# tpoisonooo/how-to-optimize-gemm

Hardware: NVIDIA H100
Metric: SGEMM GFLOP/s (square N=4096 point of the 256..4096 sweep) (higher is better)
Workload: dtype f16x2(scaled split-f32)

## Files before the change

how-to-optimize-gemm_b200/csrc/capi.cu:

```cuda
#include "../../include/b200gemm.h"

#include <cuda.h>
#include <cuda_runtime.h>
#include <stdio.h>
#include <stdlib.h>
#include <string.h>

#include <atomic>
#include <mutex>
#include <vector>

#include "gemm_ffma.cuh"
#include "gemm_generic.cuh"
#include "gemm_mxf4.cuh"
#include "gemm_tc.cuh"

using namespace b200;

namespace {

std::atomic<unsigned long long> g_launches{0};
int g_split_tail = 1;

struct KernelTimer {
// ... 2 lines not shown
  int n = 0;
  cudaEvent_t ev[CAP][2] = {};
  void begin(cudaStream_t st) {
    if (!on || n >= CAP) return;
    if (!ev[n][0]) { cudaEventCreate(&ev[n][0]); cudaEventCreate(&ev[n][1]); }
    cudaEventRecord(ev[n][0], st);
  }
  void end(cudaStream_t st) {
    if (!on || n >= CAP) return;
    cudaEventRecord(ev[n][1], st);
    n++;
  }
} g_ktimer;
std::atomic<int> g_default_f32_mode{-1};
thread_local const char* t_last_kernel = "none";
struct Schedule { int tiles = 0, split = 0, full_tiles = 0, ctas = 0; };
thread_local Schedule t_last_schedule;
int g_dbg_b_lbo = 0, g_dbg_b_sbo = 0;

struct Call {
  cudaStream_t st = nullptr;
  int acc = 0;
  int axpby = 0;
  float alpha = 1.f, beta = 0.f;
  const void* bias = nullptr;
  int act = -1;
  int sm_reserve = 0;
  bool epi() const { return act >= 0; }
};

constexpr int kFlagSlots = 16;
struct Scratch { void* p = nullptr; size_t bytes = 0; };
struct HostPipe {
  bool ready = false;
  cudaStream_t h2d = nullptr, comp = nullptr, d2h = nullptr;
  cudaEvent_t in[8] = {}, done[8] = {};
  cudaError_t init() {
    if (ready) return cudaSuccess;
    cudaError_t e;
    if ((e = cudaStreamCreateWithFlags(&h2d, cudaStreamNonBlocking)) != cudaSuccess) return e;
    if ((e = cudaStreamCreateWithFlags(&comp, cudaStreamNonBlocking)) != cudaSuccess) return e;
    if ((e = cudaStreamCreateWithFlags(&d2h, cudaStreamNonBlocking)) != cudaSuccess) return e;
    for (int i = 0; i < 8; i++) {
      if ((e = cudaEventCreateWithFlags(&in[i], cudaEventDisableTiming)) != cudaSuccess) return e;
      if ((e = cudaEventCreateWithFlags(&done[i], cudaEventDisableTiming)) != cudaSuccess) return e;
    }
    ready = true;
    return cudaSuccess;
  }
};
struct DevCtx {
  int ok = 0;
  int sms = 0;
  int dev = -1;
  int* flags = nullptr;
  std::mutex flag_mu;
  unsigned flag_slot = 0;
  struct FlagUser {
    cudaStream_t st = nullptr;
    cudaEvent_t ev = nullptr;
    bool used = false;
  } flag_user[kFlagSlots];
  std::mutex ws_mu;
  Scratch ws;
  cudaEvent_t ws_event = nullptr;
  cudaStream_t ws_stream = nullptr;
  bool ws_busy = false;
  struct MaxBuf {
    unsigned slot = 0;
    float* buf = nullptr;
    size_t cap = 0;
    int dirty[2] = {0, 0};
  } cmax, amax;
  cudaStream_t aux = nullptr;
  cudaEvent_t aux_fork = nullptr, aux_join = nullptr;
  std::mutex host_mu;
  Scratch scr[4];
  HostPipe pipe;
  std::vector<const void*> attr_done;
};
constexpr int kMaxDevices = 64;
DevCtx g_ctx[kMaxDevices];
std::mutex g_mu;

typedef CUresult (*EncodeTiledFn)(CUtensorMap*, CUtensorMapDataType, cuuint32_t, void*,
                                  const cuuint64_t*, const cuuint64_t*, const cuuint32_t*,
                                  const cuuint32_t*, CUtensorMapInterleave, CUtensorMapSwizzle,
                                  CUtensorMapL2promotion, CUtensorMapFloatOOBfill);
EncodeTiledFn g_encode = nullptr;

thread_local DevCtx* t_ctx = nullptr;
thread_local int t_bound_dev = -1;

int ensure_device() {
  int dev = -1;
  if (cudaGetDevice(&dev) != cudaSuccess || dev < 0 || dev >= kMaxDevices) { cudaGetLastError(); t_ctx = nullptr; return B200_ERR_NO_DEVICE; }
  if (t_bound_dev != dev) {
    if (cudaSetDevice(dev) != cudaSuccess) { cudaGetLastError(); t_ctx = nullptr; return B200_ERR_NO_DEVICE; }
    t_bound_dev = dev;
  }
  DevCtx* c = &g_ctx[dev];
  t_ctx = c;
  if (c->ok == 1) return 0;
  std::lock_guard<std::mutex> lk(g_mu);
  if (c->ok == 1) return 0;
  cudaDeviceProp prop;
  if (cudaGetDeviceProperties(&prop, dev) != cudaSuccess) { cudaGetLastError(); c->ok = -1; return B200_ERR_NO_DEVICE; }
  if (prop.major != 9) { c->ok = -1; return B200_ERR_NO_DEVICE; }
  if (!g_encode) {
    void* fn = nullptr;
    cudaDriverEntryPointQueryResult qres;
    if (cudaGetDriverEntryPoint("cuTensorMapEncodeTiled", &fn, cudaEnableDefault, &qres) != cudaSuccess ||
        qres != cudaDriverEntryPointSuccess || !fn) {
      cudaGetLastError();
      c->ok = -1;
      return B200_ERR_NO_DEVICE;
    }
    g_encode = reinterpret_cast<EncodeTiledFn>(fn);
  }
  if (!c->flags) {
    if (cudaMalloc(&c->flags, kFlagSlots * 1024 * sizeof(int)) != cudaSuccess ||
        cudaMemset(c->flags, 0, kFlagSlots * 1024 * sizeof(int)) != cudaSuccess) {
      cudaGetLastError(); c->flags = nullptr; c->ok = -1; return B200_ERR_NO_DEVICE;
    }
  }
  if (!c->ws_event && cudaEventCreateWithFlags(&c->ws_event, cudaEventDisableTiming) != cudaSuccess) {
    cudaGetLastError(); c->ok = -1; return B200_ERR_NO_DEVICE;
  }
  for (auto& u : c->flag_user)
    if (!u.ev && cudaEventCreateWithFlags(&u.ev, cudaEventDisableTiming) != cudaSuccess) {
      cudaGetLastError(); u.ev = nullptr; c->ok = -1; return B200_ERR_NO_DEVICE;
    }
  c->dev = dev;
  c->sms = prop.multiProcessorCount;
  c->ok = 1;
  return 0;
}

template <typename Kern>
int ensure_smem_attr(Kern kern, int bytes) {
  const void* key = reinterpret_cast<const void*>(kern);
  {
    std::lock_guard<std::mutex> lk(g_mu);
    for (const void* k : t_ctx->attr_done) if (k == key) return 0;
  }
  cudaError_t e = cudaFuncSetAttribute(kern, cudaFuncAttributeMaxDynamicSharedMemorySize, bytes);
  if (e != cudaSuccess) { cudaGetLastError(); return (int)e; }
  std::lock_guard<std::mutex> lk(g_mu);
  t_ctx->attr_done.push_back(key);
  return 0;
}

struct MapKey {
  const void* ptr; int dtype; unsigned long long d0, d1, ld_bytes; unsigned b0, b1; int swz; int dev;
  unsigned long long d2, d2_bytes;
  bool operator==(const MapKey& o) const {
    return ptr == o.ptr && dtype == o.dtype && d0 == o.d0 && d1 == o.d1 && ld_bytes == o.ld_bytes &&
           b0 == o.b0 && b1 == o.b1 && swz == o.swz && dev == o.dev && d2 == o.d2 && d2_bytes == o.d2_bytes;
  }
};
struct MapEntry { MapKey key; CUtensorMap map; };
std::vector<MapEntry> g_maps;
size_t g_map_next = 0;
constexpr size_t kMapCache = 64;

int get_map(CUtensorMap* out, const void* ptr, CUtensorMapDataType dt, int elem_bytes,
            unsigned long long inner, unsigned long long rows, unsigned long long ld_bytes,
            unsigned box_inner, unsigned box_rows, int swizzle ,
            unsigned long long entries = 0, unsigned long long entry_bytes = 0) {
  MapKey key{ptr, (int)dt, inner, rows, ld_bytes, box_inner, box_rows, swizzle, t_ctx->dev, entries, entry_bytes};
  std::lock_guard<std::mutex> lk(g_mu);
  for (auto& e : g_maps)
    if (e.key == key) { *out = e.map; return 0; }
  cuuint64_t dims[3] = {inner, rows, entries};
  cuuint64_t strides[2] = {ld_bytes, entry_bytes};
  cuuint32_t box[3] = {box_inner, box_rows, 1};
  cuuint32_t estr[3] = {1, 1, 1};
  CUtensorMap m;
  CUresult r = g_encode(&m, dt, entries ? 3 : 2, const_cast<void*>(ptr), dims, strides, box, estr,
                        CU_TENSOR_MAP_INTERLEAVE_NONE,
                        swizzle == 1 ? CU_TENSOR_MAP_SWIZZLE_128B
                        : swizzle == 2 ? CU_TENSOR_MAP_SWIZZLE_128B_ATOM_32B
                        : swizzle == 3 ? CU_TENSOR_MAP_SWIZZLE_64B : CU_TENSOR_MAP_SWIZZLE_NONE,
                        CU_TENSOR_MAP_L2_PROMOTION_L2_256B, CU_TENSOR_MAP_FLOAT_OOB_FILL_NONE);
  (void)elem_bytes;
  if (r != CUDA_SUCCESS) return B200_ERR_TENSORMAP;
  if (g_maps.size() < kMapCache) g_maps.push_back({key, m});
  else { g_maps[g_map_next] = {key, m}; g_map_next = (g_map_next + 1) % kMapCache; }
  *out = m;
  return 0;
}

inline bool aligned16(const void* p) { return (reinterpret_cast<uintptr_t>(p) & 15) == 0; }

int check_args(int m, int n, int k, const void* A, int lda, const void* B, int ldb, const void* C, int ldc,
               int op_a = B200_OP_N, int op_b = B200_OP_N) {
  if ((op_a != B200_OP_N && op_a != B200_OP_T) || (op_b != B200_OP_N && op_b != B200_OP_T)) return B200_ERR_BAD_ARG;
  if (m < 0 || n < 0 || k < 0) return B200_ERR_BAD_ARG;
  if (m == 0 || n == 0) return 1;
  if (!C || ldc < n) return B200_ERR_BAD_ARG;
  if (k > 0 && (!A || !B || lda < (op_a ? m : k) || ldb < (op_b ? k : n))) return B200_ERR_BAD_ARG;
  return 0;
}

int last_launch_status() {
  cudaError_t e = cudaPeekAtLastError();
  if (e != cudaSuccess) { cudaGetLastError(); return (int)e; }
  return 0;
}

int g_pdl = 1;
int g_prepass_fork = 1;
template <typename... KArgs, typename... Args>
cudaError_t launch_pdl(void (*kern)(KArgs...), dim3 grid, dim3 block, size_t smem, cudaStream_t st, int cluster, Args&&... args) {
  cudaLaunchConfig_t cfg = {};
  cfg.gridDim = grid; cfg.blockDim = block; cfg.dynamicSmemBytes = smem; cfg.stream = st;
  cudaLaunchAttribute at[2];
  int n = 0;
  if (cluster > 1) {
    at[n].id = cudaLaunchAttributeClusterDimension;
    at[n].val.clusterDim.x = cluster; at[n].val.clusterDim.y = 1; at[n].val.clusterDim.z = 1;
    n++;
  }
  if (g_pdl) {
    at[n].id = cudaLaunchAttributeProgrammaticStreamSerialization;
    at[n].val.programmaticStreamSerializationAllowed = 1;
    n++;
  }
  cfg.attrs = at; cfg.numAttrs = n;
  return cudaLaunchKernelEx(&cfg, kern, std::forward<Args>(args)...);
}

template <typename T>
int launch_zero(int m, int n, T* C, int ldc, cudaStream_t st) {
  dim3 grid((n + 255) / 256, m < 4096 ? m : 4096);
  fill_zero_kernel<T><<<grid, 256, 0, st>>>(m, n, C, ldc);
  g_launches++;
  t_last_kernel = "fill_zero";
  return last_launch_status();
}

template <typename InT, typename OutT>
int launch_generic(int op_a, int op_b, int m, int n, int k, const void* A, int lda, const void* B, int ldb, void* C,
                   int ldc, const char* name, const Call& c) {
  dim3 grid((n + 63) / 64, (m + 63) / 64);
  const long long a_rs = op_a ? 1 : lda, a_cs = op_a ? lda : 1, b_rs = op_b ? 1 : ldb, b_cs = op_b ? ldb : 1;
  gemm_generic_kernel<InT, OutT><<<grid, 256, 0, c.st>>>(m, n, k, static_cast<const InT*>(A), a_rs, a_cs,
                                                         static_cast<const InT*>(B), b_rs, b_cs, static_cast<OutT*>(C), ldc,
                                                         c.acc, nullptr, nullptr, c.axpby, c.alpha, c.beta,
                                                         static_cast<const InT*>(c.bias), c.act);
  g_launches++;
  t_last_kernel = name;
  return last_launch_status();
}

int launch_generic_requant(int m, int n, int k, const int8_t* A, int lda, const int8_t* B, int ldb, int8_t* C,
                           int ldc, const float* scales, const float* bias, cudaStream_t st) {
  dim3 grid((n + 63) / 64, (m + 63) / 64);
  gemm_generic_kernel<int8_t, int8_t><<<grid, 256, 0, st>>>(m, n, k, A, lda, 1, B, ldb, 1, C, ldc, 0, scales, bias);
  g_launches++;
  t_last_kernel = "generic_s8_requant_64x64";
  return last_launch_status();
}

int take_flag_slot(cudaStream_t st, int** flags, DevCtx::FlagUser** user) {
// ... 351 lines not shown
  if (ws.rc) return ws.rc;
  uint16_t* pA = reinterpret_cast<uint16_t*>(ws.base());
  const uint16_t* pB = prepB ? prepB : reinterpret_cast<uint16_t*>(ws.base() + round1024(ga.bytes(NP)));
  const SplitJob ja{A, lda, ga.rows, ga.cols, pA, ga.pitch, ga.plane_rows},
                 jb{B, ldb, gb.rows, gb.cols, const_cast<uint16_t*>(pB), gb.pitch, gb.plane_rows};
  if (int rc = launch_split<NP>(ja, jb, prepB ? 1 : 2, c.st)) return rc;
  using Prod = typename std::conditional<NP == 3, ProdX3, ProdX2>::type;
  return with_layout(op_a, op_b, [&](auto L) {
    using Lay = decltype(L);
    return launch_tc<KIND_F16, 128, NP == 3 ? 4 : 6, float, Prod, 64, Lay::AL, Lay::BL>(
        m, n, k, pA, ga.pitch, NP * ga.plane_rows, ga.plane_rows, pB, gb.pitch, NP * gb.plane_rows, gb.plane_rows, C, ldc,
        (NP == 3 ? kNamesBf16x3 : kNamesBf16x2)[Lay::idx][2], c, g_split_chunk_k[NP == 3 ? 0 : 1]);
  });
}

struct F16Operand {
  const uint16_t* planes;
  long long pitch;
  int plane_rows;
  const float* maxv;
};

int launch_f16_split_rows(const float* A, long long lda, int rows, int cols, float* rmax, uint16_t* planes,
                          long long pitch, int plane_rows, cudaStream_t st) {
  int blocks = (plane_rows + 7) / 8;
  const int cap = t_ctx->sms * 16;
  if (blocks > cap) blocks = cap;
  if (blocks < 1) blocks = 1;
  if (cols <= 1024) launch_pdl(split_f16_rows_kernel<4>, dim3(blocks), dim3(256), 0, st, 1, A, (long long)lda, rows, cols, rmax, planes, pitch, plane_rows);
  else if (cols <= 2048) launch_pdl(split_f16_rows_kernel<8>, dim3(blocks), dim3(256), 0, st, 1, A, (long long)lda, rows, cols, rmax, planes, pitch, plane_rows);
  else if (cols <= 4096) launch_pdl(split_f16_rows_kernel<16>, dim3(blocks), dim3(256), 0, st, 1, A, (long long)lda, rows, cols, rmax, planes, pitch, plane_rows);
  else launch_pdl(split_f16_rows_kernel<0>, dim3(blocks), dim3(256), 0, st, 1, A, (long long)lda, rows, cols, rmax, planes, pitch, plane_rows);
  g_launches++;
  return last_launch_status();
}

int launch_f16_split_cols(const float* B, long long ldb, int rows, int cols, float* cmax, uint16_t* planes,
                          long long pitch, int plane_rows, float* zero_buf, int zero_n, cudaStream_t st) {
  launch_pdl(col_absmax_kernel, dim3((cols + 1023) / 1024, (rows + 15) / 16), dim3(256), 0, st, 1, B, (long long)ldb, rows, cols,
             reinterpret_cast<unsigned int*>(cmax));
  const int gx = (int)((pitch + 2047) / 2048);
  int gy = (t_ctx->sms * 8 + gx - 1) / gx;
  if (gy > (plane_rows + 1) / 2) gy = (plane_rows + 1) / 2;
  if (gy < 1) gy = 1;
  if (zero_buf && zero_n > gx * 2048) {
    cudaMemsetAsync(zero_buf, 0, (size_t)zero_n * 4, st);
    zero_buf = nullptr;
  }
  launch_pdl(split_f16_cols_kernel, dim3(gx, gy), dim3(256), 0, st, 1, B, (long long)ldb, rows, cols, (const float*)cmax, planes, pitch, plane_rows, zero_buf, zero_n);
  g_launches += 2;
  return last_launch_status();
}

int gemm_f16x2_core(int op_a, int op_b, int m, int n, int k, const F16Operand& a, const F16Operand& b, float* C, int ldc,
                    const Call& c) {
  constexpr int NP = 2;
  return with_layout(op_a, op_b, [&](auto L) {
    using Lay = decltype(L);
    return launch_tc<KIND_FP16, 128, 6, float, ProdX2, 64, Lay::AL, Lay::BL>(
        m, n, k, a.planes, a.pitch, NP * a.plane_rows, a.plane_rows, b.planes, b.pitch, NP * b.plane_rows, b.plane_rows, C,
        ldc, kNamesF16x2[Lay::idx][2], c, g_split_chunk_k[2], a.maxv, b.maxv);
  });
}

int cmax_reserve(DevCtx::MaxBuf& mb, int n, float** cur, float** other, int* other_dirty) {
  if (mb.cap < (size_t)n) {
    size_t cap = mb.cap ? 2 * mb.cap : 16384;
    if (cap < (size_t)n) cap = (size_t)n;
    if (mb.buf) { cudaDeviceSynchronize(); cudaFree(mb.buf); }
    mb.buf = nullptr; mb.cap = 0;
    cudaError_t e = cudaMalloc(&mb.buf, 2 * cap * sizeof(float));
    if (e == cudaSuccess) e = cudaMemset(mb.buf, 0, 2 * cap * sizeof(float));
    if (e != cudaSuccess) { cudaGetLastError(); return (int)e; }
    mb.cap = cap;
    mb.dirty[0] = mb.dirty[1] = 0;
  }
  const unsigned slot = mb.slot++ & 1u;
  *cur = mb.buf + slot * mb.cap;
  *other = mb.buf + (slot ^ 1u) * mb.cap;
  *other_dirty = mb.dirty[slot ^ 1u];
  mb.dirty[slot ^ 1u] = 0;
  mb.dirty[slot] = n;
  return 0;
}

struct F16Ws {
  PlaneGeom ga, gb;
  size_t a_off, r_off, rb_off, total;
};
F16Ws f16x2_ws(int op_a, int op_b, int m, int n, int k, bool prepA, bool prepB) {
  F16Ws w{geom_a(op_a, m, k), geom_b(op_b, k, n)};
  w.a_off = round1024(prepA ? 0 : w.ga.bytes(2));
  w.r_off = round1024(w.a_off + (prepB ? 0 : w.gb.bytes(2)));
  const size_t ra = prepA || op_a ? 0 : (size_t)m * 4;
  w.rb_off = round1024(w.r_off + ra);
  w.total = prepB || !op_b ? w.r_off + ra : w.rb_off + (size_t)n * 4;
  return w;
}

int gemm_f32_split_f16(int op_a, int op_b, int m, int n, int k, const float* A, int lda, const float* B, int ldb, float* C,
                       int ldc, const F16Operand* prepA, const F16Operand* prepB, const Call& c) {
  if (prepA && prepB) return gemm_f16x2_core(B200_OP_N, B200_OP_N, m, n, k, *prepA, *prepB, C, ldc, c);
  const F16Ws w = f16x2_ws(op_a, op_b, m, n, k, prepA != nullptr, prepB != nullptr);
  const PlaneGeom &ga = w.ga, &gb = w.gb;
  WsLease ws(w.total, c.st);
  if (ws.rc) return ws.rc;
  uint8_t* base = ws.base();
  F16Operand oa, ob;
  DevCtx* dc = t_ctx;
  const bool fork = !prepA && !prepB && g_prepass_fork && (double)m * k + (double)k * n >= 4.0e6;
  cudaStream_t sb = c.st;
  if (fork) {
    if (!dc->aux) {
      if (cudaStreamCreateWithFlags(&dc->aux, cudaStreamNonBlocking) != cudaSuccess ||
          cudaEventCreateWithFlags(&dc->aux_fork, cudaEventDisableTiming) != cudaSuccess ||
          cudaEventCreateWithFlags(&dc->aux_join, cudaEventDisableTiming) != cudaSuccess) { cudaGetLastError(); return B200_ERR_NO_DEVICE; }
    }
    cudaEventRecord(dc->aux_fork, c.st);
    cudaStreamWaitEvent(dc->aux, dc->aux_fork, 0);
    sb = dc->aux;
  }
  if (prepB) ob = *prepB;
  else if (op_b) {
    uint16_t* pB = reinterpret_cast<uint16_t*>(base + w.a_off);
    float* bmax = reinterpret_cast<float*>(base + w.rb_off);
    if (int rc = launch_f16_split_rows(B, ldb, n, k, bmax, pB, gb.pitch, gb.plane_rows, sb)) return rc;
    ob = F16Operand{pB, gb.pitch, gb.plane_rows, bmax};
  } else {
    uint16_t* pB = reinterpret_cast<uint16_t*>(base + w.a_off);
    float *cmax, *other;
    int other_dirty;
    if (int rc = cmax_reserve(dc->cmax, n, &cmax, &other, &other_dirty)) return rc;
    if (int rc = launch_f16_split_cols(B, ldb, k, n, cmax, pB, gb.pitch, gb.plane_rows, other, other_dirty, sb)) return rc;
    ob = F16Operand{pB, gb.pitch, gb.plane_rows, cmax};
  }
  if (prepA) oa = *prepA;
  else if (op_a) {
    uint16_t* pA = reinterpret_cast<uint16_t*>(base);
    float *amax, *other;
    int other_dirty;
    if (int rc = cmax_reserve(dc->amax, m, &amax, &other, &other_dirty)) return rc;
    if (int rc = launch_f16_split_cols(A, lda, k, m, amax, pA, ga.pitch, ga.plane_rows, other, other_dirty, c.st)) return rc;
    oa = F16Operand{pA, ga.pitch, ga.plane_rows, amax};
  } else {
    uint16_t* pA = reinterpret_cast<uint16_t*>(base);
    float* rmax = reinterpret_cast<float*>(base + w.r_off);
    if (int rc = launch_f16_split_rows(A, lda, m, k, rmax, pA, ga.pitch, ga.plane_rows, c.st)) return rc;
    oa = F16Operand{pA, ga.pitch, ga.plane_rows, rmax};
  }
  if (fork) {
    cudaEventRecord(dc->aux_join, dc->aux);
    cudaStreamWaitEvent(c.st, dc->aux_join, 0);
  }
  return gemm_f16x2_core(op_a, op_b, m, n, k, oa, ob, C, ldc, c);
}

template <class Cfg, class Kern>
int launch_ffma(Kern kern, int ctas_per_sm, const char* name, int m, int n, int k, const float* A, int lda,
                const float* B, int ldb, float* C, int ldc, const Call& c) {
  CUtensorMap tmA, tmB;
  int rc = get_map(&tmA, A, CU_TENSOR_MAP_DATA_TYPE_FLOAT32, 4, k, m, (unsigned long long)lda * 4, Cfg::BK, Cfg::BM, 1);
  if (rc) return rc;
  rc = get_map(&tmB, B, CU_TENSOR_MAP_DATA_TYPE_FLOAT32, 4, n, k, (unsigned long long)ldb * 4, Cfg::BN, Cfg::BK, 0);
// ... 366 lines not shown
  if (k == 0 || alpha == 0.f) return c32 ? degenerate_grouped<float>(n, C, ldc, gr, c) : degenerate_grouped<E>(n, C, ldc, gr, c);
  if (!tma_ok(A, lda, B, ldb, 2) || (groups > 1 && !batch_tma_ok(stride_b, b_rows, ldb, 2))) {
    if (c32) return launch_generic_grouped<E, float>(op_b, n, k, A, lda, B, ldb, C, ldc, gr, K16::kGenericGrp, c);
    return launch_generic_grouped<E, E>(op_b, n, k, A, lda, B, ldb, C, ldc, gr, K16::kGenericGrp, c);
  }
  if (c32) return tc16_grouped<KIND, float>(op_b, n, k, A, lda, B, ldb, C, ldc, gr, c);
  return tc16_grouped<KIND, typename K16::Out16>(op_b, n, k, A, lda, B, ldb, C, ldc, gr, c);
}

static_assert(ACT_NONE == B200_ACT_NONE && ACT_RELU == B200_ACT_RELU && ACT_GELU == B200_ACT_GELU &&
              ACT_GELU_TANH == B200_ACT_GELU_TANH, "EpiAct follows the header's codes");

int gemm_s8(int op_a, int op_b, int m, int n, int k, const int8_t* A, int lda, const int8_t* B, int ldb, int32_t* C,
            int ldc, cudaStream_t st) {
  int rc = check_args(m, n, k, A, lda, B, ldb, C, ldc, op_a, op_b);
  if (rc == 1) return 0;
  if (rc) return rc;
  if ((rc = ensure_device())) return rc;
  Call c{st};
  if (k == 0) return launch_zero<int32_t>(m, n, C, ldc, st);
  if (!tma_ok(A, lda, B, ldb, 1))
    return launch_generic<int8_t, int32_t>(op_a, op_b, m, n, k, A, lda, B, ldb, C, ldc, "generic_s8_64x64", c);
  return tc_s8(op_a, op_b, m, n, k, A, lda, B, ldb, C, ldc, c);
}

}

extern "C" {

const char* b200_gemm_version(void) { return "b200gemm 0.3 (sm_90a; wgmma+TMA)"; }

int b200_gemm_device_ok(void) { return ensure_device(); }

const char* b200_gemm_strerror(int code) {
  switch (code) {
    case B200_OK: return "ok";
    case B200_ERR_BAD_ARG: return "bad argument";
    case B200_ERR_NO_DEVICE: return "no usable sm_90 CUDA device (there is no CPU fallback)";
    case B200_ERR_UNSUPPORTED: return "mode not supported for these operands";
    case B200_ERR_TENSORMAP: return "cuTensorMapEncodeTiled failed";
    case B200_ERR_NCCL: return "NCCL failure (b200_nccl_last_error has the text)";
    default: return code > 0 ? cudaGetErrorString((cudaError_t)code) : "unknown";
  }
}

const char* b200_gemm_last_kernel(void) { return t_last_kernel; }
unsigned long long b200_gemm_launch_count(void) { return g_launches.load(); }
int b200_gemm_default_f32_mode(void) { return resolve_f32_mode(B200_F32_AUTO); }
void b200_gemm_set_default_f32_mode(int mode) {
  if (mode >= 0 && mode != B200_F32_AUTO && mode <= B200_F32_F16X2) g_default_f32_mode.store(mode);
}
void b200_gemm_debug_set_b_desc(int lbo_bytes, int sbo_bytes) { g_dbg_b_lbo = lbo_bytes; g_dbg_b_sbo = sbo_bytes; }
void b200_gemm_debug_set_bn(int bn) { g_force_bn = bn; }
void b200_gemm_debug_set_pdl(int v) { g_pdl = (v & 1) != 0; g_prepass_fork = (v & 2) == 0; }
void b200_gemm_debug_set_dynamic_sched(int) {}
void b200_gemm_debug_set_cta_group(int) {}
void b200_gemm_debug_set_split_tail(int on) { g_split_tail = on; }
void b200_gemm_debug_last_schedule(int* tiles, int* split, int* full_tiles, int* ctas) {
  const Schedule& s = t_last_schedule;
  if (tiles) *tiles = s.tiles;
  if (split) *split = s.split;
  if (full_tiles) *full_tiles = s.full_tiles;
  if (ctas) *ctas = s.ctas;
}
void b200_gemm_debug_set_epilogue(int) {}
void b200_gemm_debug_set_group_rows(int rows) { g_group_rows = rows; }
void b200_gemm_debug_set_ffma_variant(int v) { g_ffma_halves = v & 1; g_ffma_fat = v < 0 ? -1 : (v >> 1) & 1; }
void b200_gemm_debug_set_split_chunk(int x3_k, int x2_k) {
  g_split_chunk_k[0] = x3_k < 0 ? kSplitChunkDefault[0] : x3_k;
  g_split_chunk_k[1] = x2_k < 0 ? kSplitChunkDefault[1] : x2_k;
  g_split_chunk_k[2] = x2_k < 0 ? kSplitChunkDefault[2] : x2_k;
}
void b200_gemm_debug_kernel_timing(int enable) { g_ktimer.on = enable != 0; g_ktimer.n = 0; }
int b200_gemm_debug_kernel_time_ms(double* sum_ms) {
  double sum = 0;
  int cnt = 0;
  for (int i = 0; i < g_ktimer.n; i++) {
    float ms = 0.f;
    if (cudaEventSynchronize(g_ktimer.ev[i][1]) == cudaSuccess &&
        cudaEventElapsedTime(&ms, g_ktimer.ev[i][0], g_ktimer.ev[i][1]) == cudaSuccess) { sum += ms; cnt++; }
  }
  cudaGetLastError();
  g_ktimer.n = 0;
  if (sum_ms) *sum_ms = sum;
  return cnt;
}

int b200_gemm_reserve_workspace(size_t bytes) {
  int rc = ensure_device();
  if (rc) return rc;
  std::lock_guard<std::mutex> wlk(t_ctx->ws_mu);
  return split_ws_reserve(bytes);
}
size_t b200_gemm_workspace_bytes_op(int op_a, int op_b, int m, int n, int k, int precision_mode) {
  if ((op_a != B200_OP_N && op_a != B200_OP_T) || (op_b != B200_OP_N && op_b != B200_OP_T)) return 0;
  if (m <= 0 || n <= 0 || k <= 0) return 0;
  size_t bytes = 0;
  for (int tma = 0; tma < 2; tma++)
    for (int general = 0; general < 2; general++) {
      const size_t b = f32_route_ws_bytes(f32_route(precision_mode, m, n, k, tma, general), op_a, op_b, m, n, k);
      if (b > bytes) bytes = b;
    }
  return bytes;
}
size_t b200_gemm_workspace_bytes(int m, int n, int k, int precision_mode) {
  return b200_gemm_workspace_bytes_op(B200_OP_N, B200_OP_N, m, n, k, precision_mode);
}
// ... 400 lines not shown
```

how-to-optimize-gemm_b200/csrc/gemm_tc.cuh:

```cuda
#pragma once
#include <cuda_fp16.h>
#include <string.h>
#include <type_traits>

#include "ptx.cuh"
#include "wgmma.cuh"

namespace b200 {

enum Layout { LAYOUT_K = 0, LAYOUT_MN = 1 };

template <int KIND> struct KindTraits;
template <> struct KindTraits<KIND_F16>  { static constexpr int ELEM = 2; static constexpr int B_LAYOUT = LAYOUT_MN; };
template <> struct KindTraits<KIND_FP16> { static constexpr int ELEM = 2; static constexpr int B_LAYOUT = LAYOUT_MN; };
template <> struct KindTraits<KIND_TF32> { static constexpr int ELEM = 4; static constexpr int B_LAYOUT = LAYOUT_K; };
template <> struct KindTraits<KIND_I8>   { static constexpr int ELEM = 1; static constexpr int B_LAYOUT = LAYOUT_K; };

struct ProdSingle {
  static constexpr int N = 1, NPA = 1, NPB = 1;
  __host__ __device__ static constexpr int ia(int) { return 0; }
  __host__ __device__ static constexpr int ib(int) { return 0; }
};
struct ProdX3 {
  static constexpr int N = 6, NPA = 3, NPB = 3;
// ... 813 lines not shown
          const float4 v0 = __ldcs(reinterpret_cast<const float4*>(s));
          const float4 v1 = __ldcs(reinterpret_cast<const float4*>(s) + 1);
          x[u][0] = v0.x; x[u][1] = v0.y; x[u][2] = v0.z; x[u][3] = v0.w;
          x[u][4] = v1.x; x[u][5] = v1.y; x[u][6] = v1.z; x[u][7] = v1.w;
        } else {
#pragma unroll
          for (int e = 0; e < 8; e++)
            if (c + e < cols) x[u][e] = s[e];
        }
      }
    }
#pragma unroll
    for (int u = 0; u < 2; u++) {
      const int r = r0 + u;
      if (r >= plane_rows) break;
#pragma unroll
      for (int pl = 0; pl < NP; pl++) {
        uint32_t w[4];
#pragma unroll
        for (int e = 0; e < 4; e++) w[e] = bf16_plane2(x[u][2 * e], x[u][2 * e + 1]);
        *reinterpret_cast<uint4*>(dst + ((long long)pl * plane_rows + r) * dld + c) = make_uint4(w[0], w[1], w[2], w[3]);
      }
    }
  }
}


__device__ __forceinline__ void split_f16x8(const float (&x)[8], uint4& h1, uint4& h2) {
  uint32_t a[4], b[4];
#pragma unroll
  for (int e = 0; e < 4; e++) {
    const __half2 p = __floats2half2_rn(x[2 * e], x[2 * e + 1]);
    const float2 pf = __half22float2(p);
    const __half2 q = __floats2half2_rn(x[2 * e] - pf.x, x[2 * e + 1] - pf.y);
    a[e] = *reinterpret_cast<const uint32_t*>(&p);
    b[e] = *reinterpret_cast<const uint32_t*>(&q);
  }
  h1 = make_uint4(a[0], a[1], a[2], a[3]);
  h2 = make_uint4(b[0], b[1], b[2], b[3]);
}
__device__ __forceinline__ void load8(const float* __restrict__ s, int c, int cols, bool vec, float (&x)[8]) {
  if (vec && c + 8 <= cols) {
    const float4 v0 = __ldg(reinterpret_cast<const float4*>(s + c));
    const float4 v1 = __ldg(reinterpret_cast<const float4*>(s + c) + 1);
    x[0] = v0.x; x[1] = v0.y; x[2] = v0.z; x[3] = v0.w;
    x[4] = v1.x; x[5] = v1.y; x[6] = v1.z; x[7] = v1.w;
  } else {
#pragma unroll
    for (int e = 0; e < 8; e++) x[e] = c + e < cols ? __ldg(s + c + e) : 0.f;
  }
}

template <int VPL>
__global__ void __launch_bounds__(256) split_f16_rows_kernel(const float* __restrict__ src, long long ld, int rows,
                                                             int cols, float* __restrict__ rmax,
                                                             uint16_t* __restrict__ dst, long long dld, int plane_rows) {
  griddep_launch();
  griddep_wait();
  const int lane = threadIdx.x & 31;
  const int nwarps = (gridDim.x * blockDim.x) >> 5;
  const bool vec = (ld & 3) == 0 && (reinterpret_cast<uintptr_t>(src) & 15) == 0;
  for (int r = (blockIdx.x * blockDim.x + threadIdx.x) >> 5; r < plane_rows; r += nwarps) {
    uint16_t* d1 = dst + (long long)r * dld;
    uint16_t* d2 = dst + ((long long)plane_rows + r) * dld;
    if (r >= rows) {
      for (int c = lane * 8; c < dld; c += 256) {
        *reinterpret_cast<uint4*>(d1 + c) = make_uint4(0, 0, 0, 0);
        *reinterpret_cast<uint4*>(d2 + c) = make_uint4(0, 0, 0, 0);
      }
      continue;
    }
    const float* s = src + (long long)r * ld;
    float mx = 0.f;
    if constexpr (VPL > 0) {
      float x[VPL][8];
#pragma unroll
      for (int j = 0; j < VPL; j++) {
        const int c = (j * 32 + lane) * 8;
#pragma unroll
        for (int e = 0; e < 8; e++) x[j][e] = 0.f;
        if (c < cols) load8(s, c, cols, vec, x[j]);
#pragma unroll
        for (int e = 0; e < 8; e++) mx = fmaxf(mx, fabsf(x[j][e]));
      }
#pragma unroll
      for (int o = 16; o > 0; o >>= 1) mx = fmaxf(mx, __shfl_xor_sync(0xffffffffu, mx, o));
      if (lane == 0) rmax[r] = mx;
      const int ex = -pow2_exp(mx);
#pragma unroll
      for (int j = 0; j < VPL; j++) {
        const int c = (j * 32 + lane) * 8;
        if (c < dld) {
#pragma unroll
          for (int e = 0; e < 8; e++) x[j][e] = scale_pow2(x[j][e], ex);
          uint4 h1, h2;
          split_f16x8(x[j], h1, h2);
          *reinterpret_cast<uint4*>(d1 + c) = h1;
          *reinterpret_cast<uint4*>(d2 + c) = h2;
        }
      }
    } else {
      for (int c0 = lane * 8; c0 < cols; c0 += 1024) {
        float x[4][8];
#pragma unroll
        for (int u = 0; u < 4; u++) {
          const int c = c0 + u * 256;
#pragma unroll
          for (int e = 0; e < 8; e++) x[u][e] = 0.f;
          if (c < cols) load8(s, c, cols, vec, x[u]);
#pragma unroll
          for (int e = 0; e < 8; e++) mx = fmaxf(mx, fabsf(x[u][e]));
        }
      }
#pragma unroll
      for (int o = 16; o > 0; o >>= 1) mx = fmaxf(mx, __shfl_xor_sync(0xffffffffu, mx, o));
      if (lane == 0) rmax[r] = mx;
      const int ex = -pow2_exp(mx);
      for (int c0 = lane * 8; c0 < dld; c0 += 512) {
        float x[2][8];
#pragma unroll
        for (int u = 0; u < 2; u++) {
          const int c = c0 + u * 256;
#pragma unroll
          for (int e = 0; e < 8; e++) x[u][e] = 0.f;
          if (c < cols) load8(s, c, cols, vec, x[u]);
        }
#pragma unroll
        for (int u = 0; u < 2; u++) {
          const int c = c0 + u * 256;
          if (c < dld) {
#pragma unroll
            for (int e = 0; e < 8; e++) x[u][e] = scale_pow2(x[u][e], ex);
            uint4 h1, h2;
            split_f16x8(x[u], h1, h2);
            *reinterpret_cast<uint4*>(d1 + c) = h1;
            *reinterpret_cast<uint4*>(d2 + c) = h2;
          }
        }
      }
    }
  }
}

__global__ void __launch_bounds__(256) col_absmax_kernel(const float* __restrict__ src, long long ld, int rows,
                                                         int cols, unsigned int* __restrict__ out) {
  constexpr int ROWS = 16;
  griddep_launch();
  griddep_wait();
  const int c = blockIdx.x * 1024 + threadIdx.x * 4;
  if (c >= cols) return;
  const int r0 = blockIdx.y * ROWS, r1 = min(r0 + ROWS, rows);
  const bool vec = (ld & 3) == 0 && (reinterpret_cast<uintptr_t>(src) & 15) == 0 && c + 4 <= cols;
  float4 mx = make_float4(0.f, 0.f, 0.f, 0.f);
  if (vec) {
#pragma unroll 16
    for (int r = r0; r < r1; r++) {
      const float4 v = __ldg(reinterpret_cast<const float4*>(src + (long long)r * ld + c));
      mx.x = fmaxf(mx.x, fabsf(v.x)); mx.y = fmaxf(mx.y, fabsf(v.y));
      mx.z = fmaxf(mx.z, fabsf(v.z)); mx.w = fmaxf(mx.w, fabsf(v.w));
    }
  } else {
    for (int r = r0; r < r1; r++) {
      const float* s = src + (long long)r * ld + c;
      mx.x = fmaxf(mx.x, fabsf(s[0]));
      if (c + 1 < cols) mx.y = fmaxf(mx.y, fabsf(s[1]));
      if (c + 2 < cols) mx.z = fmaxf(mx.z, fabsf(s[2]));
      if (c + 3 < cols) mx.w = fmaxf(mx.w, fabsf(s[3]));
    }
  }
  const float m4[4] = {mx.x, mx.y, mx.z, mx.w};
#pragma unroll
  for (int e = 0; e < 4; e++)
    if (c + e < cols && __float_as_uint(m4[e]) > __ldcg(out + c + e)) atomicMax(out + c + e, __float_as_uint(m4[e]));
}

__global__ void __launch_bounds__(256) split_f16_cols_kernel(const float* __restrict__ src, long long ld, int rows,
                                                             int cols, const float* __restrict__ cmax,
                                                             uint16_t* __restrict__ dst, long long dld, int plane_rows,
                                                             float* __restrict__ zero_buf, int zero_n) {
  griddep_launch();
  griddep_wait();
  const int c = (int)(blockIdx.x * 256 + threadIdx.x) * 8;
  if (blockIdx.y == 0 && zero_buf != nullptr) {
#pragma unroll
    for (int e = 0; e < 8; e++)
      if (c + e < zero_n) zero_buf[c + e] = 0.f;
  }
  if (c >= dld) return;
  const bool vec = (ld & 3) == 0 && (reinterpret_cast<uintptr_t>(src) & 15) == 0;
  int ex[8];
#pragma unroll
  for (int e = 0; e < 8; e++) ex[e] = c + e < cols ? -pow2_exp(__ldg(cmax + c + e)) : 0;
  for (int r0 = blockIdx.y * 2; r0 < plane_rows; r0 += gridDim.y * 2) {
    float x[2][8];
#pragma unroll
    for (int u = 0; u < 2; u++) {
      const int r = r0 + u;
#pragma unroll
      for (int e = 0; e < 8; e++) x[u][e] = 0.f;
      if (r < rows) load8(src + (long long)r * ld, c, cols, vec, x[u]);
    }
#pragma unroll
    for (int u = 0; u < 2; u++) {
      const int r = r0 + u;
      if (r >= plane_rows) break;
#pragma unroll
      for (int e = 0; e < 8; e++) x[u][e] = scale_pow2(x[u][e], ex[e]);
      uint4 h1, h2;
      split_f16x8(x[u], h1, h2);
      *reinterpret_cast<uint4*>(dst + (long long)r * dld + c) = h1;
      *reinterpret_cast<uint4*>(dst + ((long long)plane_rows + r) * dld + c) = h2;
    }
  }
}

}
```

how-to-optimize-gemm_b200/csrc/ptx.cuh:

```cuda
#pragma once
#include <cuda.h>
#include <cuda_runtime.h>
#include <math.h>
#include <stdint.h>

namespace b200 {

__device__ __forceinline__ uint32_t smem_u32(const void* p) {
  return static_cast<uint32_t>(__cvta_generic_to_shared(p));
}

__device__ __forceinline__ void mbar_init(uint32_t bar, uint32_t count) {
  asm volatile("mbarrier.init.shared::cta.b64 [%0], %1;" ::"r"(bar), "r"(count) : "memory");
}
__device__ __forceinline__ void fence_barrier_init() {
  asm volatile("fence.mbarrier_init.release.cluster;" ::: "memory");
}
__device__ __forceinline__ void fence_proxy_async() {
  asm volatile("fence.proxy.async.shared::cta;" ::: "memory");
}
__device__ __forceinline__ void mbar_arrive_expect_tx(uint32_t bar, uint32_t bytes) {
  asm volatile("mbarrier.arrive.expect_tx.shared::cta.b64 _, [%0], %1;" ::"r"(bar), "r"(bytes)
               : "memory");
}
// ... 44 lines not shown
      "cp.async.bulk.tensor.2d.shared::cluster.global.tile.mbarrier::complete_tx::bytes"
      ".L2::cache_hint [%0], [%1, {%3, %4}], [%2], %5;"
      ::"r"(dst_smem), "l"(reinterpret_cast<uint64_t>(m)), "r"(bar), "r"(c0), "r"(c1), "l"(policy)
      : "memory");
}

enum MmaKind { KIND_F16 = 0 , KIND_TF32 = 1, KIND_I8 = 2, KIND_FP16 = 3  };
enum Swz { SWZ_128B = 1, SWZ_64B = 2 };

__device__ __forceinline__ uint64_t make_sdesc(uint32_t smem_addr, uint32_t lbo_bytes, uint32_t sbo_bytes, uint32_t swz) {
  uint64_t d = 0;
  d |= (uint64_t)((smem_addr & 0x3FFFF) >> 4);
  d |= (uint64_t)((lbo_bytes >> 4) & 0x3FFF) << 16;
  d |= (uint64_t)((sbo_bytes >> 4) & 0x3FFF) << 32;
  d |= (uint64_t)swz << 62;
  return d;
}

__device__ __forceinline__ int32_t requant_s8(int32_t acc, float scale, float bias, bool has_bias) {
  float f = __fmul_rn(__int2float_rn(acc), scale);
  if (has_bias) f = __fadd_rn(f, bias);
  const float g = fminf(fmaxf(f, -200.0f), 200.0f);
  const float magic = 12582912.0f;
  float r = __fadd_rn(__fadd_rn(g, magic), -magic);
  if (fabsf(__fadd_rn(g, -r)) == 0.5f && fabsf(r) < fabsf(g)) r = __fadd_rn(r, copysignf(1.0f, g));
  r = fminf(fmaxf(r, -128.0f), 127.0f);
  const int32_t q = __float_as_int(__fadd_rn(r, magic)) - 0x4B400000;
  return f != f ? 0 : q;
}

enum EpiAct { ACT_NONE = 0, ACT_RELU = 1, ACT_GELU = 2, ACT_GELU_TANH = 3 };
template <int ACT>
__device__ __forceinline__ float epi_act(float t) {
  if constexpr (ACT == ACT_RELU) {
    return t < 0.f ? 0.f : t;
  } else if constexpr (ACT == ACT_GELU) {
    const float g = __fmul_rn(__fmul_rn(0.5f, t), erfcf(__fmul_rn(-0.707106781186547524f, t)));
    return t == -INFINITY ? -0.f : g;
  } else if constexpr (ACT == ACT_GELU_TANH) {
    const float u = __fmul_rn(0.797884560802865356f, __fmaf_rn(__fmul_rn(0.044715f, t), __fmul_rn(t, t), t));
    const float g = __fmul_rn(__fmul_rn(0.5f, t), __fadd_rn(1.f, tanhf(u)));
    return t == -INFINITY ? -0.f : g;
  } else {
    return t;
  }
}

template <int N> __device__ __forceinline__ void setmaxnreg_inc() { asm volatile("setmaxnreg.inc.sync.aligned.u32 %0;" ::"n"(N)); }
template <int N> __device__ __forceinline__ void setmaxnreg_dec() { asm volatile("setmaxnreg.dec.sync.aligned.u32 %0;" ::"n"(N)); }

__device__ __forceinline__ void griddep_launch() { asm volatile("griddepcontrol.launch_dependents;" ::: "memory"); }
__device__ __forceinline__ void griddep_wait() { asm volatile("griddepcontrol.wait;" ::: "memory"); }

__device__ __forceinline__ bool elect_one() {
  uint32_t pred;
  asm volatile("{\n\t.reg .pred p;\n\telect.sync _|p, 0xffffffff;\n\tselp.b32 %0, 1, 0, p;\n\t}" : "=r"(pred));
  return pred != 0;
}

constexpr int kMaxGroups = 1024;

__device__ __forceinline__ void group_table(const int* __restrict__ offs, int groups, int total_m, int rows, int* end,
                                            int* block) {
  for (int i = threadIdx.x; i < groups; i += blockDim.x) end[i + 1] = offs[i];
  __syncthreads();
  if (threadIdx.x < 32) {
    const int lane = threadIdx.x;
    int run_end = 0, run_blocks = 0;
    for (int base = 0; base < groups; base += 32) {
      const int g = base + lane;
      int e = max(g < groups ? end[g + 1] : 0, run_end);
#pragma unroll
      for (int d = 1; d < 32; d <<= 1) {
        const int o = __shfl_up_sync(0xffffffffu, e, d);
        if (lane >= d) e = max(e, o);
      }
      e = min(e, total_m);
      int prev = __shfl_up_sync(0xffffffffu, e, 1);
      if (lane == 0) prev = run_end;
      int b = (e - prev) / rows + ((e - prev) % rows != 0);
#pragma unroll
      for (int d = 1; d < 32; d <<= 1) {
        const int o = __shfl_up_sync(0xffffffffu, b, d);
        if (lane >= d) b += o;
      }
      if (g < groups) { end[g + 1] = e; block[g + 1] = run_blocks + b; }
      run_end = __shfl_sync(0xffffffffu, e, 31);
      run_blocks += __shfl_sync(0xffffffffu, b, 31);
    }
    if (lane == 0) { end[0] = 0; block[0] = 0; }
  }
  __syncthreads();
}

__device__ __forceinline__ int group_of(const int* block, int groups, int q) {
  int lo = 0, hi = groups - 1;
  while (lo < hi) {
    const int mid = (lo + hi + 1) >> 1;
    if (block[mid] <= q) lo = mid;
    else hi = mid - 1;
  }
  return lo;
}

}
```

Before: 184,600.

## Fuse A and B f16x2 split prepasses into one paired cluster kernel

```diff
diff --git a/how-to-optimize-gemm_b200/csrc/capi.cu b/how-to-optimize-gemm_b200/csrc/capi.cu
--- a/how-to-optimize-gemm_b200/csrc/capi.cu
+++ b/how-to-optimize-gemm_b200/csrc/capi.cu
@@ -78,6 +78,7 @@
 struct DevCtx {
   int ok = 0;
   int sms = 0;
+  int smem_optin = 0;
   int dev = -1;
   int* flags = nullptr;
   std::mutex flag_mu;
@@ -159,6 +160,7 @@
     }
   c->dev = dev;
   c->sms = prop.multiProcessorCount;
+  c->smem_optin = (int)prop.sharedMemPerBlockOptin;
   c->ok = 1;
   return 0;
 }
@@ -237,6 +239,7 @@
 
 int g_pdl = 1;
 int g_prepass_fork = 1;
+int g_prepass_pair = 1;
 template <typename... KArgs, typename... Args>
 cudaError_t launch_pdl(void (*kern)(KArgs...), dim3 grid, dim3 block, size_t smem, cudaStream_t st, int cluster, Args&&... args) {
   cudaLaunchConfig_t cfg = {};
@@ -694,6 +697,39 @@
   return last_launch_status();
 }
 
+constexpr int kStripW = 32, kStripCluster = 4;
+using PairKern = void (*)(const F16SplitJob, const F16SplitJob);
+PairKern pair_kernel(int k) {
+  if (k <= 1024) return split_f16x2_pair_kernel<4, kStripW>;
+  if (k <= 2048) return split_f16x2_pair_kernel<8, kStripW>;
+  if (k <= 4096) return split_f16x2_pair_kernel<16, kStripW>;
+  return split_f16x2_pair_kernel<0, kStripW>;
+}
+int pair_smem(PairKern kern, int plane_rows, int* dyn_cap) {
+  cudaFuncAttributes fa;
+  if (cudaFuncGetAttributes(&fa, kern) != cudaSuccess) { cudaGetLastError(); return -1; }
+  *dyn_cap = t_ctx->smem_optin - (int)fa.sharedSizeBytes;
+  const long long dyn = (long long)((plane_rows + kStripCluster - 1) / kStripCluster) * kStripW * 4;
+  return dyn <= *dyn_cap ? (int)dyn : -1;
+}
+int pair_blocks(const F16SplitJob& j) {
+  if (j.strip) return (j.cols + kStripW - 1) / kStripW * kStripCluster;
+  int blocks = (j.plane_rows + 7) / 8;
+  if (blocks > t_ctx->sms * 16) blocks = t_ctx->sms * 16;
+  return (blocks + kStripCluster - 1) / kStripCluster * kStripCluster;
+}
+int launch_f16x2_pair(PairKern kern, F16SplitJob ja, F16SplitJob jb, int smem, int dyn_cap, cudaStream_t st) {
+  if (!ja.strip && jb.strip) std::swap(ja, jb);
+  ja.blocks = pair_blocks(ja);
+  jb.blocks = pair_blocks(jb);
+  const bool strips = ja.strip || jb.strip;
+  if (strips)
+    if (int rc = ensure_smem_attr(kern, dyn_cap)) return rc;
+  launch_pdl(kern, dim3(ja.blocks + jb.blocks), dim3(256), strips ? (size_t)smem : 0, st, strips ? kStripCluster : 1, ja, jb);
+  g_launches++;
+  return last_launch_status();
+}
+
 int gemm_f16x2_core(int op_a, int op_b, int m, int n, int k, const F16Operand& a, const F16Operand& b, float* C, int ldc,
                     const Call& c) {
   constexpr int NP = 2;
@@ -750,7 +786,41 @@
   uint8_t* base = ws.base();
   F16Operand oa, ob;
   DevCtx* dc = t_ctx;
-  const bool fork = !prepA && !prepB && g_prepass_fork && (double)m * k + (double)k * n >= 4.0e6;
+  const bool big = (double)m * k + (double)k * n >= 4.0e6;
+  if (!prepA && !prepB && g_prepass_pair && big) {
+    const bool strips = op_a || !op_b;
+    const PairKern kern = pair_kernel(k);
+    int dyn_cap = 0;
+    const int smem = strips ? pair_smem(kern, b_plane_rows(k), &dyn_cap) : 0;
+    if (smem >= 0) {
+      uint16_t* pA = reinterpret_cast<uint16_t*>(base);
+      uint16_t* pB = reinterpret_cast<uint16_t*>(base + w.a_off);
+      F16SplitJob ja, jb;
+      if (op_a) {
+        float *amax, *other;
+        int other_dirty;
+        if (int rc = cmax_reserve(dc->amax, m, &amax, &other, &other_dirty)) return rc;
+        ja = F16SplitJob{A, lda, k, m, amax, pA, ga.pitch, ga.plane_rows, 0, 1, other, other_dirty};
+      } else {
+        float* rmax = reinterpret_cast<float*>(base + w.r_off);
+        ja = F16SplitJob{A, lda, m, k, rmax, pA, ga.pitch, ga.plane_rows, 0, 0, nullptr, 0};
+      }
+      if (op_b) {
+        float* bmax = reinterpret_cast<float*>(base + w.rb_off);
+        jb = F16SplitJob{B, ldb, n, k, bmax, pB, gb.pitch, gb.plane_rows, 0, 0, nullptr, 0};
+      } else {
+        float *cmax, *other;
+        int other_dirty;
+        if (int rc = cmax_reserve(dc->cmax, n, &cmax, &other, &other_dirty)) return rc;
+        jb = F16SplitJob{B, ldb, k, n, cmax, pB, gb.pitch, gb.plane_rows, 0, 1, other, other_dirty};
+      }
+      if (int rc = launch_f16x2_pair(kern, ja, jb, smem, dyn_cap, c.st)) return rc;
+      oa = F16Operand{pA, ga.pitch, ga.plane_rows, ja.maxv};
+      ob = F16Operand{pB, gb.pitch, gb.plane_rows, jb.maxv};
+      return gemm_f16x2_core(op_a, op_b, m, n, k, oa, ob, C, ldc, c);
+    }
+  }
+  const bool fork = !prepA && !prepB && g_prepass_fork && big;
   cudaStream_t sb = c.st;
   if (fork) {
     if (!dc->aux) {
@@ -1223,7 +1293,7 @@
 }
 void b200_gemm_debug_set_b_desc(int lbo_bytes, int sbo_bytes) { g_dbg_b_lbo = lbo_bytes; g_dbg_b_sbo = sbo_bytes; }
 void b200_gemm_debug_set_bn(int bn) { g_force_bn = bn; }
-void b200_gemm_debug_set_pdl(int v) { g_pdl = (v & 1) != 0; g_prepass_fork = (v & 2) == 0; }
+void b200_gemm_debug_set_pdl(int v) { g_pdl = (v & 1) != 0; g_prepass_fork = (v & 2) == 0; g_prepass_pair = (v & 4) == 0; }
 void b200_gemm_debug_set_dynamic_sched(int) {}
 void b200_gemm_debug_set_cta_group(int) {}
 void b200_gemm_debug_set_split_tail(int on) { g_split_tail = on; }
diff --git a/how-to-optimize-gemm_b200/csrc/gemm_tc.cuh b/how-to-optimize-gemm_b200/csrc/gemm_tc.cuh
--- a/how-to-optimize-gemm_b200/csrc/gemm_tc.cuh
+++ b/how-to-optimize-gemm_b200/csrc/gemm_tc.cuh
@@ -889,15 +889,12 @@
 }
 
 template <int VPL>
-__global__ void __launch_bounds__(256) split_f16_rows_kernel(const float* __restrict__ src, long long ld, int rows,
-                                                             int cols, float* __restrict__ rmax,
-                                                             uint16_t* __restrict__ dst, long long dld, int plane_rows) {
-  griddep_launch();
-  griddep_wait();
+__device__ __forceinline__ void split_f16_rows(const float* __restrict__ src, long long ld, int rows, int cols,
+                                               float* __restrict__ rmax, uint16_t* __restrict__ dst, long long dld,
+                                               int plane_rows, int warp, int nwarps) {
   const int lane = threadIdx.x & 31;
-  const int nwarps = (gridDim.x * blockDim.x) >> 5;
   const bool vec = (ld & 3) == 0 && (reinterpret_cast<uintptr_t>(src) & 15) == 0;
-  for (int r = (blockIdx.x * blockDim.x + threadIdx.x) >> 5; r < plane_rows; r += nwarps) {
+  for (int r = warp; r < plane_rows; r += nwarps) {
     uint16_t* d1 = dst + (long long)r * dld;
     uint16_t* d2 = dst + ((long long)plane_rows + r) * dld;
     if (r >= rows) {
@@ -977,6 +974,15 @@
       }
     }
   }
+}
+template <int VPL>
+__global__ void __launch_bounds__(256) split_f16_rows_kernel(const float* __restrict__ src, long long ld, int rows,
+                                                             int cols, float* __restrict__ rmax,
+                                                             uint16_t* __restrict__ dst, long long dld, int plane_rows) {
+  griddep_launch();
+  griddep_wait();
+  split_f16_rows<VPL>(src, ld, rows, cols, rmax, dst, dld, plane_rows, (blockIdx.x * blockDim.x + threadIdx.x) >> 5,
+                      (gridDim.x * blockDim.x) >> 5);
 }
 
 __global__ void __launch_bounds__(256) col_absmax_kernel(const float* __restrict__ src, long long ld, int rows,
@@ -1051,4 +1057,128 @@
   }
 }
 
-}
+struct F16SplitJob {
+  const float* src;
+  long long ld;
+  int rows, cols;
+  float* maxv;
+  uint16_t* dst;
+  long long dld;
+  int plane_rows;
+  int blocks;
+  int strip;
+  float* zero_buf;
+  int zero_n;
+};
+
+template <int W>
+__device__ __forceinline__ void split_f16_strip(const F16SplitJob& j, int b, float* __restrict__ tile) {
+  constexpr int G = W / 4;
+  constexpr int RG = 256 / G;
+  constexpr int Q = W / 8;
+  constexpr int U = 16;
+  __shared__ float part[RG * W];
+  __shared__ float pmax[W], cmax[W];
+  const uint32_t ncta = cluster_nctarank(), rank = cluster_ctarank();
+  const int t = threadIdx.x;
+  const int c0 = (int)(b / ncta) * W;
+  const int rc = (int)((j.plane_rows + ncta - 1) / ncta);
+  const int r0 = (int)rank * rc, r1 = min(r0 + rc, j.plane_rows), rl = min(r1, j.rows);
+  {
+    const int cg = t % G, c = c0 + cg * 4;
+    const bool vec = (j.ld & 3) == 0 && (reinterpret_cast<uintptr_t>(j.src) & 15) == 0 && c + 4 <= j.cols;
+    float4 mx = make_float4(0.f, 0.f, 0.f, 0.f);
+    for (int rb = r0 + t / G; rb < rl; rb += RG * U) {
+      float4 v[U];
+#pragma unroll
+      for (int u = 0; u < U; u++) {
+        const int r = rb + u * RG;
+        v[u] = make_float4(0.f, 0.f, 0.f, 0.f);
+        if (r < rl) {
+          const float* s = j.src + (long long)r * j.ld + c;
+          if (vec) {
+            v[u] = __ldg(reinterpret_cast<const float4*>(s));
+          } else {
+            if (c < j.cols) v[u].x = __ldg(s);
+            if (c + 1 < j.cols) v[u].y = __ldg(s + 1);
+            if (c + 2 < j.cols) v[u].z = __ldg(s + 2);
+            if (c + 3 < j.cols) v[u].w = __ldg(s + 3);
+          }
+        }
+      }
+#pragma unroll
+      for (int u = 0; u < U; u++) {
+        const int r = rb + u * RG;
+        if (r < rl) {
+          *reinterpret_cast<float4*>(tile + (r - r0) * W + cg * 4) = v[u];
+          mx.x = fmaxf(mx.x, fabsf(v[u].x)); mx.y = fmaxf(mx.y, fabsf(v[u].y));
+          mx.z = fmaxf(mx.z, fabsf(v[u].z)); mx.w = fmaxf(mx.w, fabsf(v[u].w));
+        }
+      }
+    }
+    *reinterpret_cast<float4*>(part + (t / G) * W + cg * 4) = mx;
+  }
+  __syncthreads();
+  if (t < W) {
+    float m = 0.f;
+#pragma unroll 8
+    for (int i = 0; i < RG; i++) m = fmaxf(m, part[i * W + t]);
+    pmax[t] = m;
+  }
+  cluster_arrive();
+  cluster_wait();
+  if (t < W) {
+    float m = 0.f;
+    for (uint32_t q = 0; q < ncta; q++) m = fmaxf(m, ld_dsmem(pmax + t, q));
+    cmax[t] = m;
+    if (rank == 0 && c0 + t < j.cols) j.maxv[c0 + t] = m;
+  }
+  cluster_arrive();
+  __syncthreads();
+  const int ch = t % Q, c = c0 + ch * 8;
+  if (c < j.dld) {
+    int ex[8];
+#pragma unroll
+    for (int e = 0; e < 8; e++) ex[e] = c + e < j.cols ? -pow2_exp(cmax[ch * 8 + e]) : 0;
+    for (int r = r0 + t / Q; r < r1; r += 256 / Q) {
+      float x[8];
+      if (r < rl) {
+        const float4 v0 = *reinterpret_cast<const float4*>(tile + (r - r0) * W + ch * 8);
+        const float4 v1 = *reinterpret_cast<const float4*>(tile + (r - r0) * W + ch * 8 + 4);
+        x[0] = v0.x; x[1] = v0.y; x[2] = v0.z; x[3] = v0.w;
+        x[4] = v1.x; x[5] = v1.y; x[6] = v1.z; x[7] = v1.w;
+      } else {
+#pragma unroll
+        for (int e = 0; e < 8; e++) x[e] = 0.f;
+      }
+#pragma unroll
+      for (int e = 0; e < 8; e++) x[e] = scale_pow2(x[e], ex[e]);
+      uint4 h1, h2;
+      split_f16x8(x, h1, h2);
+      *reinterpret_cast<uint4*>(j.dst + (long long)r * j.dld + c) = h1;
+      *reinterpret_cast<uint4*>(j.dst + ((long long)j.plane_rows + r) * j.dld + c) = h2;
+    }
+  }
+  cluster_wait();
+}
+
+template <int VPL, int W>
+__global__ void __launch_bounds__(256) split_f16x2_pair_kernel(const F16SplitJob j0, const F16SplitJob j1) {
+  extern __shared__ float4 f16_strip_tile[];
+  griddep_launch();
+  griddep_wait();
+  const int nthreads = gridDim.x * blockDim.x, tid = blockIdx.x * blockDim.x + threadIdx.x;
+  for (int i = tid; i < j0.zero_n; i += nthreads) j0.zero_buf[i] = 0.f;
+  for (int i = tid; i < j1.zero_n; i += nthreads) j1.zero_buf[i] = 0.f;
+  auto run = [&](const F16SplitJob& j, int b) {
+    if (j.strip)
+      split_f16_strip<W>(j, b, reinterpret_cast<float*>(f16_strip_tile));
+    else
+      split_f16_rows<VPL>(j.src, j.ld, j.rows, j.cols, j.maxv, j.dst, j.dld, j.plane_rows,
+                          (b * blockDim.x + threadIdx.x) >> 5, (j.blocks * blockDim.x) >> 5);
+  };
+  if ((int)blockIdx.x < j0.blocks) run(j0, blockIdx.x);
+  else run(j1, blockIdx.x - j0.blocks);
+}
+
+}
diff --git a/how-to-optimize-gemm_b200/csrc/ptx.cuh b/how-to-optimize-gemm_b200/csrc/ptx.cuh
--- a/how-to-optimize-gemm_b200/csrc/ptx.cuh
+++ b/how-to-optimize-gemm_b200/csrc/ptx.cuh
@@ -120,6 +120,26 @@
 __device__ __forceinline__ void griddep_launch() { asm volatile("griddepcontrol.launch_dependents;" ::: "memory"); }
 __device__ __forceinline__ void griddep_wait() { asm volatile("griddepcontrol.wait;" ::: "memory"); }
 
+__device__ __forceinline__ uint32_t cluster_ctarank() {
+  uint32_t r;
+  asm volatile("mov.u32 %0, %%cluster_ctarank;" : "=r"(r));
+  return r;
+}
+__device__ __forceinline__ uint32_t cluster_nctarank() {
+  uint32_t r;
+  asm volatile("mov.u32 %0, %%cluster_nctarank;" : "=r"(r));
+  return r;
+}
+__device__ __forceinline__ void cluster_arrive() { asm volatile("barrier.cluster.arrive;" ::: "memory"); }
+__device__ __forceinline__ void cluster_wait() { asm volatile("barrier.cluster.wait;" ::: "memory"); }
+__device__ __forceinline__ float ld_dsmem(const float* p, uint32_t rank) {
+  uint32_t a;
+  float v;
+  asm volatile("mapa.shared::cluster.u32 %0, %1, %2;" : "=r"(a) : "r"(smem_u32(p)), "r"(rank));
+  asm volatile("ld.shared::cluster.f32 %0, [%1];" : "=f"(v) : "r"(a) : "memory");
+  return v;
+}
+
 __device__ __forceinline__ bool elect_one() {
   uint32_t pred;
   asm volatile("{\n\t.reg .pred p;\n\telect.sync _|p, 0xffffffff;\n\tselp.b32 %0, 1, 0, p;\n\t}" : "=r"(pred));
```

New measurement: 188,500 (median of 6 runs). 2.1% higher.
